# fraunhoferhhi/vvenc

Measured on AMD Instinct MI355X. Metric: frames/sec + bit-exact vs CPU, 1080p/4K 10-bit preset=faster at 1/2/4/8 GPU, higher is better.
Workload: dtype i16; 1 GPU; BASELINE configs[1]: hot-path work lists RECORDED from the reference encoder (1920x1080 10-bit synthetic clip, 65 frames, preset faster; one picture per temporal layer), replayed resident in HBM: a step = one picture's integer-ME SAD windows + sub-pel SATD stages + table calls + fused TU transform/quant lists + DMVR lists on 5 HIP streams; steps follow the GOP's 1:1:2:4:8:16 layer mix from the key; hip_streams=5, sample_pairs_per_frame=175309451, coefficients_per_frame=6951461, recorded_calls_outside_the_lists=0

## Files before the change

### vvenc_amd/csrc/me.hip

```cpp
#include <stdlib.h>
#ifndef VVHIP_ME_HU
#define VVHIP_ME_HU 2
#endif
#ifndef VVHIP_ME_STAGE_WAVES
#define VVHIP_ME_STAGE_WAVES 6
#endif
#ifndef VVHIP_ME_ITEM_WAVES
#define VVHIP_ME_ITEM_WAVES 8
#endif
#include <string.h>
#include <algorithm>
#include <vector>
#include "common.h"

struct vvhip_me_plan
{
  int bitDepth = 0, nCands = 0, nStages = 0, nItems = 0, nMaskItems = 0, maxPlane = 0;
  int wavesInt = 0, wavesStage = 0, wavesItem = 0, wavesItemMain = 0, ldsInt = 0, ldsStage = 0;
  int intBig = 0, ldsIntSmall = 0;
  int intLarge = 0, ldsIntMid = 0;
  bool stageAtomic = false;
  bool intSplit = false;
  bool timing = false; hipEvent_t ev[5] = { nullptr, nullptr, nullptr, nullptr, nullptr };
  int stageSetWaves[6] = { 0, 0, 0, 0, 0, 0 }, stageSetLds[6] = { 0, 0, 0, 0, 0, 0 };
  void* d_blob = nullptr;
  const void* d_intJobs = nullptr; const void* d_cands = nullptr; const void* d_candOut = nullptr; const void* d_stageJobs = nullptr; const void* d_stageOrder = nullptr; const void* d_stageWaves = nullptr;
  const void* d_items = nullptr; const void* d_itemOrder = nullptr; const void* d_itemWaves = nullptr; const void* d_tapTables = nullptr; const void* d_maskItems = nullptr;
};

namespace {

typedef uint32_t u32x2 __attribute__( ( ext_vector_type( 2 ) ) );
typedef uint32_t u32x4 __attribute__( ( ext_vector_type( 4 ) ) );
typedef short s16x2 __attribute__( ( ext_vector_type( 2 ) ) );
struct __attribute__( ( packed, aligned( 2 ) ) ) U8  { u32x2 v; };
struct __attribute__( ( packed, aligned( 2 ) ) ) U16 { u32x4 v; };
#define ME_GLOBAL __attribute__( ( address_space( 1 ) ) )
__device__ __forceinline__ u32x2 ld8( const int16_t* p )  { return ( ( const ME_GLOBAL U8* ) p )->v; }
__device__ __forceinline__ u32x4 ld16( const int16_t* p ) { return ( ( const ME_GLOBAL U16* ) p )->v; }
__device__ __forceinline__ u32x4 ld16o( const char* base, uint32_t byteOff ) { return reinterpret_cast<const U16*>( base + byteOff )->v; }
__device__ __forceinline__ u32x2 ld8o( const char* base, uint32_t byteOff ) { return reinterpret_cast<const U8*>( base + byteOff )->v; }
__device__ __forceinline__ int lo16( uint32_t v ) { return ( int ) ( int16_t ) ( v & 0xffffu ); }
__device__ __forceinline__ int hi16( uint32_t v ) { return ( int ) ( ( int32_t ) v >> 16 ); }
__device__ __forceinline__ uint32_t pkAdd( uint32_t a, uint32_t b ) { return __builtin_bit_cast( uint32_t, __builtin_bit_cast( s16x2, a ) + __builtin_bit_cast( s16x2, b ) ); }
__device__ __forceinline__ uint32_t pkSub( uint32_t a, uint32_t b ) { return __builtin_bit_cast( uint32_t, __builtin_bit_cast( s16x2, a ) - __builtin_bit_cast( s16x2, b ) ); }
__device__ __forceinline__ uint32_t pack2( int lo, int hi ) { return ( ( uint32_t ) lo & 0xffffu ) | ( ( uint32_t ) hi << 16 ); }
constexpr uint32_t BIAS = 0x80008000u;

struct MePlanes { const int16_t* p[16]; int stride[16]; };

struct IntJob   { int32_t orgOff, refOff; int16_t w, h; uint8_t orgPlane, refPlane, subShift, pad; int16_t minDx, minDy, winW, winH; int32_t firstCand, nCand; };
struct PlanCand { int16_t dx, dy; uint32_t out; };
struct WaveSpan { int32_t first, count; };
struct StageUnit
{
  vvhip_me_stage_job j;
  int16_t hx[3]; uint8_t nHor, nPos;
  uint8_t cnt0, cnt1, cnt2, pad;
  int32_t order;
  int32_t pos[9];
  int32_t pad2[3];
};
static_assert( sizeof( StageUnit ) == 88, "StageUnit layout" );
struct MeArgs
{
  const IntJob* intJobs; const PlanCand* cands; const int32_t* candOut; int wavesInt;
  const StageUnit* stageUnits; const WaveSpan* stageWaves; int wavesStage;
  const int32_t* tapTables;
  const vvhip_me_item* items; const int32_t* itemOrder; const WaveSpan* itemWaves; int wavesItem;
  const vvhip_me_mask_item* maskItems;
  uint64_t* candCost; uint64_t* stageCost; uint64_t* itemCost;
  int bitDepth;
};

__device__ __forceinline__ uint32_t hadamard4x4( int ( &d )[16] )
{
#pragma unroll
  for( int r = 0; r < 4; r++ )
  {
    const int a = d[4 * r], b = d[4 * r + 1], c = d[4 * r + 2], e = d[4 * r + 3];
    const int s0 = a + b, s1 = a - b, s2 = c + e, s3 = c - e;
    d[4 * r] = s0 + s2; d[4 * r + 1] = s1 + s3; d[4 * r + 2] = s0 - s2; d[4 * r + 3] = s1 - s3;
  }
  uint32_t s = 0;
#pragma unroll
  for( int c = 0; c < 4; c++ )
  {
    const int a = d[c], b = d[4 + c], e = d[8 + c], f = d[12 + c];
    const int s0 = a + b, s1 = a - b, s2 = e + f, s3 = e - f;
    const int v0 = s0 + s2, v1 = s1 + s3, v2 = s0 - s2, v3 = s1 - s3;
    s += ( c == 0 ? ( ( uint32_t ) abs( v0 ) >> 2 ) : ( uint32_t ) abs( v0 ) ) + ( uint32_t ) abs( v1 ) + ( uint32_t ) abs( v2 ) + ( uint32_t ) abs( v3 );
  }
  return ( s + 1 ) >> 1;
}

__device__ __forceinline__ int winPitch( int winW ) { return 2 * ( ( ( winW + 3 ) >> 1 ) | 1 ); }

template<bool ONE_WAVE>
__device__ __forceinline__ void intBody( const MePlanes& P, const MeArgs& a, int wave, int16_t* lds )
{
  const IntJob j = a.intJobs[wave];
  const int tid = ONE_WAVE ? ( int ) ( threadIdx.x & 63 ) : ( int ) threadIdx.x, nthr = ONE_WAVE ? 64 : ( int ) blockDim.x, lane = tid & 63;
  const int w = j.w, ss = j.subShift, rowsEff = j.h >> ss, lpr = w >> 3, lprShift = 31 - __builtin_clz( lpr );
  const int pitch = winPitch( j.winW ), half0 = ( j.winH + 1 ) >> 1;
  int16_t* win = lds;
  int16_t* orgL = lds + ( ( j.winH * pitch + 7 ) & ~7 );
  PlanCand* candL = reinterpret_cast<PlanCand*>( orgL + rowsEff * w );
  {
    PlanCand myCand = { 0, 0, 0u };
    if( tid < j.nCand ) myCand = a.cands[j.firstCand + tid];
    const char* orgB = reinterpret_cast<const char*>( P.p[j.orgPlane] + j.orgOff );
    const int os = P.stride[j.orgPlane] ? P.stride[j.orgPlane] : w, m = rowsEff * lpr;
    u32x4 ov[4]; int oat[4];
#pragma unroll
    for( int q = 0; q < 4; q++ )
    {
      const int i = tid + nthr * q < m ? tid + nthr * q : 0, r = i >> lprShift, c = i & ( lpr - 1 );
      oat[q] = r * w + c * 8;
      ov[q] = ld16o( orgB, ( uint32_t ) ( __mul24( r << ss, os ) + c * 8 ) * 2u );
    }
    const char* refB = reinterpret_cast<const char*>( P.p[j.refPlane] + j.refOff + ( ptrdiff_t ) j.minDy * P.stride[j.refPlane] + j.minDx );
    const int cpr = ( j.winW + 2 + 7 ) >> 3, n = j.winH * cpr, rs = P.stride[j.refPlane];
    const uint32_t cprInv = ( ( 1u << 20 ) + ( uint32_t ) cpr - 1u ) / ( uint32_t ) cpr;
    for( int i0 = tid; i0 < n; i0 += 4 * nthr )
    {
      u32x4 v[4]; int at[4], cc[4];
#pragma unroll
      for( int q = 0; q < 4; q++ )
      {
        const int i = i0 + nthr * q < n ? i0 + nthr * q : i0, r = ( int ) ( __umul24( ( uint32_t ) i, cprInv ) >> 20 ), c = i - __mul24( r, cpr );
        const int dr = ss ? ( ( r & 1 ) ? half0 : 0 ) + ( r >> 1 ) : r;
        at[q] = __mul24( dr, pitch ) + c * 8; cc[q] = c;
        v[q] = ld16o( refB, ( uint32_t ) ( __mul24( r, rs ) + c * 8 ) * 2u );
      }
#pragma unroll
      for( int q = 0; q < 4; q++ )
        if( i0 + nthr * q < n )
        {
          uint32_t* d = reinterpret_cast<uint32_t*>( win + at[q] );
          const int left = ( pitch >> 1 ) - cc[q] * 4;
          d[0] = v[q].x ^ BIAS; if( left > 1 ) d[1] = v[q].y ^ BIAS; if( left > 2 ) d[2] = v[q].z ^ BIAS; if( left > 3 ) d[3] = v[q].w ^ BIAS;
        }
    }
#pragma unroll
    for( int q = 0; q < 4; q++ )
      if( tid + nthr * q < m ) { u32x4 x = ov[q]; x.x ^= BIAS; x.y ^= BIAS; x.z ^= BIAS; x.w ^= BIAS; *reinterpret_cast<u32x4*>( orgL + oat[q] ) = x; }
    for( int i0 = tid + 4 * nthr; i0 < m; i0 += nthr )
    {
      const int r = i0 >> lprShift, c = i0 & ( lpr - 1 );
      u32x4 x = ld16o( orgB, ( uint32_t ) ( __mul24( r << ss, os ) + c * 8 ) * 2u ); x.x ^= BIAS; x.y ^= BIAS; x.z ^= BIAS; x.w ^= BIAS;
      *reinterpret_cast<u32x4*>( orgL + r * w + c * 8 ) = x;
    }
    if( tid < j.nCand ) candL[tid] = myCand;
    for( int i = tid + nthr; i < j.nCand; i += nthr ) candL[i] = a.cands[j.firstCand + i];
  }
  if( ONE_WAVE ) { __builtin_amdgcn_fence( __ATOMIC_ACQ_REL, "wavefront" ); __builtin_amdgcn_wave_barrier(); }
  else __syncthreads();
  const int chunks = rowsEff * lpr;
  int lpc = 64; while( lpc > chunks ) lpc >>= 1;
  const int teams = nthr / lpc, lt = tid & ( lpc - 1 ), team = tid / lpc;
  for( int c0 = 0; c0 < j.nCand; c0 += teams )
  {
    const int ci = c0 + team;
    const bool valid = ci < j.nCand;
    const PlanCand cd = candL[valid ? ci : 0];
    const int myOut = ( valid && ( uint32_t ) lt <= ( cd.out >> 24 ) ) ? a.candOut[( cd.out & 0xffffffu ) + lt] : -1;
    const int x = cd.dx - j.minDx, y = cd.dy - j.minDy;
    const int rowBase = ss ? ( ( y & 1 ) ? half0 : 0 ) + ( y >> 1 ) : y;
    const int16_t* base = win + rowBase * pitch + ( x & ~1 );
    const uint32_t sh = ( x & 1 ) * 16;
    uint32_t sad = 0;
    const uint32_t* pc = reinterpret_cast<const uint32_t*>( base + ( lt >> lprShift ) * pitch + ( lt & ( lpr - 1 ) ) * 8 );
    const u32x4* po = reinterpret_cast<const u32x4*>( orgL + ( lt >> lprShift ) * w + ( lt & ( lpr - 1 ) ) * 8 );
    const int rowStep = lpc >> lprShift, curStep = rowStep * ( pitch >> 1 ), orgStep = rowStep * ( w >> 3 );
#pragma unroll 2
    for( int it = chunks / lpc; it > 0; it-- )
    {
      const u32x4 o = *po;
      const uint32_t v0 = pc[0], v1 = pc[1], v2 = pc[2], v3 = pc[3], v4 = pc[4];
      sad = __builtin_amdgcn_sad_u16( __builtin_amdgcn_alignbit( v1, v0, sh ), o.x, sad );
      sad = __builtin_amdgcn_sad_u16( __builtin_amdgcn_alignbit( v2, v1, sh ), o.y, sad );
      sad = __builtin_amdgcn_sad_u16( __builtin_amdgcn_alignbit( v3, v2, sh ), o.z, sad );
      sad = __builtin_amdgcn_sad_u16( __builtin_amdgcn_alignbit( v4, v3, sh ), o.w, sad );
      pc += curStep; po += orgStep;
    }
    const uint32_t t = vvhipGroupSum32( sad, lpc, lane );
    if( myOut >= 0 ) a.candCost[myOut] = ( uint64_t ) t << ss;
  }
}

static const int8_t kLuma8[9][8] = {
  { 0, 0, 0, 64, 0, 0, 0, 0 }, { 0, 1, -3, 63, 4, -2, 1, 0 }, { -1, 2, -5, 62, 8, -3, 1, 0 }, { -1, 3, -8, 60, 13, -4, 1, 0 }, { -1, 4, -10, 58, 17, -5, 1, 0 },
  { -1, 4, -11, 52, 26, -8, 3, -1 }, { -1, 3, -9, 47, 31, -10, 4, -1 }, { -1, 4, -11, 45, 34, -10, 4, -1 }, { -1, 4, -11, 40, 40, -11, 4, -1 } };
static const int8_t kLuma6[9][8] = {
  { 0, 0, 0, 64, 0, 0, 0, 0 }, { 0, 1, -3, 63, 4, -2, 1, 0 }, { 0, 1, -5, 62, 8, -3, 1, 0 }, { 0, 2, -8, 60, 13, -4, 1, 0 }, { 0, 3, -10, 58, 17, -5, 1, 0 },
  { 0, 3, -11, 52, 26, -8, 2, 0 }, { 0, 2, -9, 47, 31, -10, 3, 0 }, { 0, 3, -11, 45, 34, -10, 3, 0 }, { 0, 3, -11, 40, 40, -11, 3, 0 } };
static const int8_t kAltHpel[8] = { 0, 3, 9, 20, 20, 9, 3, 0 };
static const int8_t kChroma4[17][4] = {
  { 0, 64, 0, 0 }, { -1, 63, 2, 0 }, { -2, 62, 4, 0 }, { -2, 60, 7, -1 }, { -2, 58, 10, -2 }, { -3, 57, 12, -2 }, { -4, 56, 14, -2 }, { -4, 55, 15, -2 }, { -4, 54, 16, -2 },
  { -5, 53, 18, -2 }, { -6, 52, 20, -2 }, { -6, 49, 24, -3 }, { -6, 46, 28, -4 }, { -5, 44, 29, -4 }, { -4, 42, 30, -4 }, { -4, 39, 33, -4 }, { -4, 36, 36, -4 } };

static int stageTap( int frac, int k, int filterMode, int altHpel )
{
  if( altHpel && frac == 8 ) return kAltHpel[k];
  if( filterMode == 2 )
  {
    const int ph = frac << 1;
    return ( k < 2 || k > 5 ) ? 0 : ( ph <= 16 ? kChroma4[ph][k - 2] : kChroma4[32 - ph][5 - k] );
  }
  const int p = frac <= 8 ? frac : 16 - frac, kk = frac <= 8 ? k : 7 - k;
  return filterMode == 0 ? kLuma8[p][kk] : kLuma6[p][kk];
}

static std::vector<int32_t> stageTapTables( int bitDepth )
{
  const int headRoom = 14 - bitDepth > 2 ? 14 - bitDepth : 2, vScale = 1 << ( 10 - headRoom ), hScale = 1 << ( 2 + headRoom );
  std::vector<int32_t> tapTab( 6 * 192, 0 );
  for( int mode = 0; mode < 3; mode++ ) for( int alt = 0; alt < 2; alt++ )
  {
    int32_t* t = &tapTab[( mode * 2 + alt ) * 192];
    const int set = ( mode == 2 && !alt ) ? 0 : ( mode == 0 ? 2 : 1 ), k0 = set == 0 ? 2 : ( set == 1 ? 1 : 0 ), np = set == 0 ? 2 : ( set == 1 ? 3 : 4 );
// ... 661 lines not shown
  extern __shared__ __attribute__( ( aligned( 16 ) ) ) int16_t meLds[];
  const int blk = ( int ) blockIdx.x + blockBase;
  if( blk < nBig ) { intBody<false>( P, a, blk, meLds ); return; }
  const int wv = __builtin_amdgcn_readfirstlane( ( int ) ( threadIdx.x >> 6 ) );
  const int job = nBig + ( blk - nBig ) * 4 + wv;
  if( job < a.wavesInt ) intBody<true>( P, a, job, meLds + wv * ( ldsSmall >> 1 ) );
}

template<int WAVES, bool GEN>
__global__ void __launch_bounds__( 64 * WAVES ) __attribute__( ( amdgpu_waves_per_eu( GEN ? VVHIP_ME_ITEM_WAVES - 1 : VVHIP_ME_ITEM_WAVES, GEN ? VVHIP_ME_ITEM_WAVES - 1 : VVHIP_ME_ITEM_WAVES ) ) )
meItemKernel( MePlanes P, MeArgs a, int nItems, int firstWave, int nWaves, int spansPerWave )
{
  const int wave = ( ( int ) blockIdx.x * WAVES + __builtin_amdgcn_readfirstlane( ( int ) ( threadIdx.x >> 6 ) ) ) * spansPerWave;
  for( int q = 0; q < spansPerWave; q++ )
    if( wave + q < nWaves ) { itemBody<GEN>( P, a, firstWave + wave + q, nItems ); __builtin_amdgcn_fence( __ATOMIC_ACQ_REL, "wavefront" ); __builtin_amdgcn_wave_barrier(); }
}

std::vector<int> xcdBandOrder( int nGroups, int base )
{
  std::vector<int> perm( nGroups );
  const int q = ( nGroups + 7 ) / 8;
  int cursor[8], endOf[8];
  for( int x = 0; x < 8; x++ ) { cursor[x] = std::min( nGroups, x * q ); endOf[x] = std::min( nGroups, ( x + 1 ) * q ); }
  for( int l = 0; l < nGroups; l++ )
  {
    int x = ( base + l ) & 7;
    for( int t = 0; t < 8 && cursor[x] >= endOf[x]; t++ ) x = ( x + 1 ) & 7;
    perm[l] = cursor[x]++;
  }
  return perm;
}
bool xcdBandOn() { static const bool on = !( getenv( "VVHIP_ME_XCD_BAND" ) && atoi( getenv( "VVHIP_ME_XCD_BAND" ) ) == 0 ); return on; }

int hostWinPitch( int winW ) { return 2 * ( ( ( winW + 3 ) >> 1 ) | 1 ); }
int hostWinSamples( int winW, int winH ) { return ( winH * hostWinPitch( winW ) + 7 ) & ~7; }

}

#ifndef VVHIP_ME_KERNELS_ONLY
extern "C" {

static int mePlanCreate( vvhip_ctx* ctx, const vvhip_me_lists& L, int bit_depth, int max_window, vvhip_me_plan** out );

int vvhip_get_me_tap_tables_host( int bit_depth, int32_t* host_out )
{
  if( bit_depth < 8 || bit_depth > 10 || !host_out ) return VVHIP_E_ARG;
  const std::vector<int32_t> t = stageTapTables( bit_depth );
  memcpy( host_out, t.data(), t.size() * sizeof( int32_t ) );
  return VVHIP_OK;
}

int vvhip_me_plan_create( vvhip_ctx* ctx, const vvhip_me_int_job* int_jobs, int n_int_jobs, const vvhip_me_cand* cands, int n_cands,
                          const vvhip_me_stage_job* stage_jobs, int n_stage_jobs, const vvhip_me_item* items, int n_items, int bit_depth, int max_window, vvhip_me_plan** out )
{
  vvhip_me_lists L; L.int_jobs = int_jobs; L.n_int_jobs = n_int_jobs; L.cands = cands; L.n_cands = n_cands; L.stage_jobs = stage_jobs; L.n_stage_jobs = n_stage_jobs;
  L.items = items; L.n_items = n_items; L.mask_items = nullptr; L.n_mask_items = 0;
  return mePlanCreate( ctx, L, bit_depth, max_window, out );
}

int vvhip_me_plan_create_lists( vvhip_ctx* ctx, const vvhip_me_lists* lists, int bit_depth, int max_window, vvhip_me_plan** out )
{
  if( !ctx || !lists ) return VVHIP_E_ARG;
  return mePlanCreate( ctx, *lists, bit_depth, max_window, out );
}

static int mePlanCreate( vvhip_ctx* ctx, const vvhip_me_lists& L, int bit_depth, int max_window, vvhip_me_plan** out )
{
  if( !ctx || !out ) return VVHIP_E_ARG;
  *out = nullptr;
  const vvhip_me_int_job* int_jobs = L.int_jobs; const vvhip_me_cand* cands = L.cands; const vvhip_me_stage_job* stage_jobs = L.stage_jobs; const vvhip_me_item* items = L.items;
  const vvhip_me_mask_item* mask_items = L.mask_items;
  const int n_int_jobs = L.n_int_jobs, n_cands = L.n_cands, n_stage_jobs = L.n_stage_jobs, n_items = L.n_items, n_mask = L.n_mask_items;
  if( n_int_jobs < 0 || n_cands < 0 || n_stage_jobs < 0 || n_items < 0 || n_mask < 0 || ( n_int_jobs && ( !int_jobs || !cands ) ) || ( n_stage_jobs && !stage_jobs ) || ( n_items && !items ) || ( n_mask && !mask_items ) )
    return vvhip_fail( ctx, VVHIP_E_ARG, "vvhip_me_plan_create: bad lists" );
  if( n_cands >= ( 1 << 24 ) ) return vvhip_fail( ctx, VVHIP_E_ARG, "vvhip_me_plan_create: %d candidates (the schedule packs the output-list position into 24 bits)", n_cands );
  if( n_stage_jobs > ST_STAGE_MASK ) return vvhip_fail( ctx, VVHIP_E_ARG, "vvhip_me_plan_create: %d stage jobs (the schedule packs the stage index into 22 bits)", n_stage_jobs );
  if( bit_depth < 8 || bit_depth > 10 ) return vvhip_fail( ctx, VVHIP_E_UNSUPPORTED, "vvhip_me_plan_create: bit depth %d (the packed Hadamard tile covers <= 10)", bit_depth );
  if( max_window <= 0 ) max_window = 24;
  auto shapeOk = []( int w, int h, int minW, int minH ) { return isPow2( w ) && isPow2( h ) && w >= minW && h >= minH && w <= 128 && h <= 128; };

  std::vector<IntJob> ij; std::vector<PlanCand> pc; std::vector<int32_t> candOut;
  int ldsInt = 0;
  static const bool dedupe = !( getenv( "VVHIP_ME_DEDUPE" ) && atoi( getenv( "VVHIP_ME_DEDUPE" ) ) == 0 );
  static const int candCap = getenv( "VVHIP_ME_CAND_CAP" ) ? atoi( getenv( "VVHIP_ME_CAND_CAP" ) ) : 16;
  for( int i = 0; i < n_int_jobs; i++ )
  {
    const vvhip_me_int_job& s = int_jobs[i];
    if( !shapeOk( s.width, s.height, 8, 4 ) || s.org_plane > 15 || s.ref_plane > 15 || s.sub_shift > 1 || ( s.height >> s.sub_shift ) < 1 || s.first_cand < 0 || s.n_cand < 0 || s.first_cand + s.n_cand > n_cands )
      return vvhip_fail( ctx, VVHIP_E_ARG, "vvhip_me_plan_create: integer job %d (%dx%d, candidates %d+%d)", i, s.width, s.height, s.first_cand, s.n_cand );
    struct WinCand { int16_t dx, dy; std::vector<int32_t> outs; };
    struct Win { int x0, y0, x1, y1; std::vector<WinCand> c; };
    const int teamLanes = std::min( 64, ( s.height >> s.sub_shift ) * ( s.width >> 3 ) );
    std::vector<Win> wins;
    const int reach = std::min( max_window, s.width * s.height >= 128 * 64 ? 16 : max_window );
    for( int k = 0; k < s.n_cand; k++ )
    {
      const vvhip_me_cand& c = cands[s.first_cand + k];
      WinCand p; p.dx = c.dx; p.dy = c.dy; p.outs.assign( 1, s.first_cand + k );
      bool placed = false;
      if( dedupe )
        for( Win& wn : wins )
        {
          for( WinCand& q : wn.c ) if( q.dx == c.dx && q.dy == c.dy && ( int ) q.outs.size() < teamLanes ) { q.outs.push_back( s.first_cand + k ); placed = true; break; }
          if( placed ) break;
        }
      if( placed ) continue;
      for( Win& wn : wins )
      {
        if( ( int ) wn.c.size() >= candCap ) continue;
        const int x0 = std::min( wn.x0, ( int ) c.dx ), y0 = std::min( wn.y0, ( int ) c.dy ), x1 = std::max( wn.x1, ( int ) c.dx ), y1 = std::max( wn.y1, ( int ) c.dy );
        if( x1 - x0 <= reach && y1 - y0 <= reach ) { wn.x0 = x0; wn.y0 = y0; wn.x1 = x1; wn.y1 = y1; wn.c.push_back( p ); placed = true; break; }
      }
      if( !placed ) { Win wn; wn.x0 = wn.x1 = c.dx; wn.y0 = wn.y1 = c.dy; wn.c.push_back( p ); wins.push_back( wn ); }
    }
    for( const Win& wn : wins )
    {
      IntJob j; j.orgOff = s.org_off; j.refOff = s.ref_off; j.w = s.width; j.h = s.height; j.orgPlane = s.org_plane; j.refPlane = s.ref_plane; j.subShift = s.sub_shift; j.pad = 0;
      j.minDx = ( int16_t ) wn.x0; j.minDy = ( int16_t ) wn.y0; j.winW = ( int16_t ) ( wn.x1 - wn.x0 + s.width ); j.winH = ( int16_t ) ( wn.y1 - wn.y0 + s.height );
      j.firstCand = ( int32_t ) pc.size(); j.nCand = ( int32_t ) wn.c.size();
      for( const WinCand& q : wn.c )
      {
        PlanCand pcd; pcd.dx = q.dx; pcd.dy = q.dy; pcd.out = ( uint32_t ) candOut.size() | ( uint32_t ) ( q.outs.size() - 1 ) << 24;
        pc.push_back( pcd ); candOut.insert( candOut.end(), q.outs.begin(), q.outs.end() );
      }
      ij.push_back( j );
      ldsInt = std::max( ldsInt, ( hostWinSamples( j.winW, j.winH ) + ( s.height >> s.sub_shift ) * s.width ) * 2 + j.nCand * ( int ) sizeof( PlanCand ) );
    }
  }
  auto ldsOf = []( const IntJob& j ) { return ( hostWinSamples( j.winW, j.winH ) + ( j.h >> j.subShift ) * j.w ) * 2 + j.nCand * ( int ) sizeof( PlanCand ); };
  const int ldsSmallCap = 6 * 1024, ldsMidCap = 24 * 1024;
  const bool band = xcdBandOn();
  auto classOf = [&]( const IntJob& j ) { const int l = ldsOf( j ); return l > ldsMidCap ? 0 : ( l > ldsSmallCap ? 1 : 2 ); };
  std::stable_sort( ij.begin(), ij.end(), [&]( const IntJob& a, const IntJob& b ) { const int ca = classOf( a ), cb = classOf( b ); if( ca != cb ) return ca < cb;
                    if( band ) return a.refOff < b.refOff;
                    return ( long ) a.nCand * a.w * ( a.h >> a.subShift ) + ( long ) a.winW * a.winH > ( long ) b.nCand * b.w * ( b.h >> b.subShift ) + ( long ) b.winW * b.winH; } );
  int intLarge = 0, intBig = 0, ldsIntSmall = 0, ldsIntMid = 0;
  for( const IntJob& j : ij ) { const int c = classOf( j ); if( c == 0 ) intLarge++; if( c <= 1 ) intBig++; if( c == 1 ) ldsIntMid = std::max( ldsIntMid, ldsOf( j ) ); if( c == 2 ) ldsIntSmall = std::max( ldsIntSmall, ldsOf( j ) ); }
  if( band && !ij.empty() )
  {
    auto weightOf = []( const IntJob& j ) { return ( long ) j.nCand * j.w * ( j.h >> j.subShift ) + ( long ) j.winW * j.winH; };
    auto heavyFirstPerEighth = [&]( int begin, int n, int per ) { const int q = ( ( n + per - 1 ) / per + 7 ) / 8 * per;
      for( int x = 0; x < 8 && q; x++ ) { const int a = std::min( n, x * q ), b = std::min( n, ( x + 1 ) * q );
        std::stable_sort( ij.begin() + begin + a, ij.begin() + begin + b, [&]( const IntJob& u, const IntJob& v ) { return weightOf( u ) > weightOf( v ); } ); } };
    heavyFirstPerEighth( 0, intLarge, 1 );
    heavyFirstPerEighth( intLarge, intBig - intLarge, 1 );
    heavyFirstPerEighth( intBig, ( int ) ij.size() - intBig, 4 );
    std::vector<IntJob> src( ij );
    const std::vector<int> pl = xcdBandOrder( intLarge, 0 );
    for( int l = 0; l < intLarge; l++ ) ij[l] = src[pl[l]];
    const std::vector<int> pb = xcdBandOrder( intBig - intLarge, intLarge );
    for( int l = 0; l < intBig - intLarge; l++ ) ij[intLarge + l] = src[intLarge + pb[l]];
    const int nSmall = ( int ) src.size() - intBig, nGr = ( nSmall + 3 ) / 4;
    const std::vector<int> ps = xcdBandOrder( nGr, intBig );
    for( int l = 0, o = intBig; l < nGr; l++ ) for( int k = 0; k < 4 && ps[l] * 4 + k < nSmall; k++ ) ij[o++] = src[intBig + ps[l] * 4 + k];
  }

  std::vector<WaveSpan> stWaves;
  int ldsStage = 0;
  for( int i = 0; i < n_stage_jobs; i++ )
  {
    const vvhip_me_stage_job& s = stage_jobs[i];
    bool ok = shapeOk( s.width, s.height, 4, 4 ) && !( s.width == 4 && s.height == 4 ) && s.org_plane <= 15 && s.ref_plane <= 15 && ( s.i_frac == 1 || s.i_frac == 2 ) && s.filter_mode <= 2 &&
              ( s.func == VVHIP_DF_SAD || s.func == VVHIP_DF_HAD || s.func == VVHIP_DF_HAD_FAST ) && !( s.mask >> 9 );
    for( int k = 0; ok && k < 9; k++ )
      if( ( s.mask >> k ) & 1 )
      {
        static const int8_t rxT[9] = { 0, 0, 0, -1, 1, -1, 1, -1, 1 }, ryH[9] = { 0, -1, 1, 0, 0, -1, -1, 1, 1 }, ryQ[9] = { 0, -1, 1, -1, -1, 0, 0, 1, 1 };
        const int tx = ( rxT[k] + s.base_qx ) * s.i_frac * 4, ty = ( ( s.i_frac == 2 ? ryH[k] : ryQ[k] ) + s.base_qy ) * s.i_frac * 4;
        if( tx < -16 || tx > 16 || ty < -16 || ty > 16 ) ok = false;
      }
// ... 196 lines not shown
  }

  int maxPlane = 0;
  for( int i = 0; i < n_int_jobs; i++ ) maxPlane = std::max( maxPlane, ( int ) std::max( int_jobs[i].org_plane, int_jobs[i].ref_plane ) );
  for( int i = 0; i < n_stage_jobs; i++ ) maxPlane = std::max( maxPlane, ( int ) std::max( stage_jobs[i].org_plane, stage_jobs[i].ref_plane ) );
  for( int i = 0; i < n_items; i++ ) maxPlane = std::max( maxPlane, ( int ) std::max( items[i].org_plane, items[i].cur_plane ) );
  for( int i = 0; i < n_mask; i++ ) maxPlane = std::max( maxPlane, ( int ) std::max( mask_items[i].mask_plane, std::max( mask_items[i].org_plane, mask_items[i].cur_plane ) ) );
  std::vector<StageUnit> stUnits( stOrder.size() );
  for( size_t i = 0; i < stOrder.size(); i++ )
  {
    StageUnit& u = stUnits[i];
    memset( &u, 0, sizeof( u ) );
    u.j = stage_jobs[stOrder[i] & ST_STAGE_MASK]; u.order = stOrder[i];
    static const int8_t rxT[9] = { 0, 0, 0, -1, 1, -1, 1, -1, 1 }, ryH[9] = { 0, -1, 1, 0, 0, -1, -1, 1, 1 }, ryQ[9] = { 0, -1, 1, -1, -1, 0, 0, 1, 1 };
    int tx[9], ty[9], var[9], cnt[3] = { 0, 0, 0 }, nHor = 0, nPos = 0;
    for( int k = 0; k < 9; k++ )
    {
      if( !( ( u.j.mask >> k ) & 1 ) ) continue;
      tx[k] = ( rxT[k] + u.j.base_qx ) * u.j.i_frac * 4; ty[k] = ( ( u.j.i_frac == 2 ? ryH[k] : ryQ[k] ) + u.j.base_qy ) * u.j.i_frac * 4;
      int v = 0; while( v < nHor && u.hx[v] != tx[k] ) v++;
      if( v == nHor ) u.hx[nHor++] = ( int16_t ) tx[k];
      var[k] = v; cnt[v]++; nPos++;
    }
    u.nHor = ( uint8_t ) nHor; u.nPos = ( uint8_t ) nPos; u.cnt0 = ( uint8_t ) cnt[0]; u.cnt1 = ( uint8_t ) cnt[1]; u.cnt2 = ( uint8_t ) cnt[2];
    int slot[3] = { 0, cnt[0], cnt[0] + cnt[1] };
    for( int k = 0; k < 9; k++ ) if( ( u.j.mask >> k ) & 1 ) u.pos[slot[var[k]]++] = k | ( ( tx[k] + 64 ) << 8 ) | ( ( ty[k] + 64 ) << 20 );
  }
  std::vector<vvhip_me_item> itSorted( n_items );
  for( int i = 0; i < n_items; i++ ) itSorted[i] = items[itOrder[i]];
  std::vector<vvhip_me_mask_item> mkSorted( n_mask );
  for( int i = 0; i < n_mask; i++ ) { mkSorted[i] = mask_items[itOrder[n_items + i]]; itOrder[n_items + i] += n_items; }
  const std::vector<int32_t> tapTab = stageTapTables( bit_depth );
  auto pad = []( size_t b ) { return ( b + 255 ) & ~( size_t ) 255; };
  const size_t bInt = pad( ij.size() * sizeof( IntJob ) ), bCand = pad( pc.size() * sizeof( PlanCand ) ), bCandO = pad( candOut.size() * 4 ), bSt = pad( stUnits.size() * sizeof( StageUnit ) ),
               bStO = pad( stOrder.size() * 4 ), bStW = pad( stWaves.size() * sizeof( WaveSpan ) ), bIt = pad( ( size_t ) n_items * sizeof( vvhip_me_item ) ), bItO = pad( itOrder.size() * 4 ),
               bItW = pad( itWaves.size() * sizeof( WaveSpan ) ), bMk = pad( mkSorted.size() * sizeof( vvhip_me_mask_item ) );
  const size_t bTap = pad( tapTab.size() * 4 );
  const size_t total = bInt + bCand + bCandO + bSt + bStO + bStW + bIt + bItO + bItW + bTap + bMk + 256;
  std::vector<char> host( total, 0 );
  size_t o = 0;
  auto put = [&]( const void* src, size_t bytes, size_t padded ) { const size_t at = o; if( bytes ) memcpy( host.data() + o, src, bytes ); o += padded; return at; };
  const size_t oInt = put( ij.data(), ij.size() * sizeof( IntJob ), bInt ), oCand = put( pc.data(), pc.size() * sizeof( PlanCand ), bCand ), oCandO = put( candOut.data(), candOut.size() * 4, bCandO ),
               oSt = put( stUnits.data(), stUnits.size() * sizeof( StageUnit ), bSt ), oStO = put( stOrder.data(), stOrder.size() * 4, bStO ),
               oStW = put( stWaves.data(), stWaves.size() * sizeof( WaveSpan ), bStW ), oIt = put( itSorted.data(), ( size_t ) n_items * sizeof( vvhip_me_item ), bIt ),
               oItO = put( itOrder.data(), itOrder.size() * 4, bItO ), oItW = put( itWaves.data(), itWaves.size() * sizeof( WaveSpan ), bItW ), oTap = put( tapTab.data(), tapTab.size() * 4, bTap ),
               oMk = put( mkSorted.data(), mkSorted.size() * sizeof( vvhip_me_mask_item ), bMk );
  vvhip_me_plan* p = new vvhip_me_plan;
  hipError_t e = hipMalloc( &p->d_blob, total );
  if( e != hipSuccess ) { delete p; return vvhip_fail( ctx, VVHIP_E_NOMEM, "vvhip_me_plan_create: hipMalloc( %zu ): %s", total, hipGetErrorString( e ) ); }
  e = hipMemcpyAsync( p->d_blob, host.data(), total, hipMemcpyHostToDevice, ctx->stream );
  if( e == hipSuccess ) e = hipStreamSynchronize( ctx->stream );
  if( e != hipSuccess ) { ( void ) hipFree( p->d_blob ); delete p; return vvhip_fail( ctx, VVHIP_E_HIP, "vvhip_me_plan_create: upload: %s", hipGetErrorString( e ) ); }
  char* b = static_cast<char*>( p->d_blob );
  p->d_intJobs = b + oInt; p->d_cands = b + oCand; p->d_candOut = b + oCandO; p->d_stageJobs = b + oSt; p->d_stageOrder = b + oStO; p->d_stageWaves = b + oStW; p->d_items = b + oIt; p->d_itemOrder = b + oItO; p->d_itemWaves = b + oItW; p->d_tapTables = b + oTap; p->d_maskItems = b + oMk;
  p->bitDepth = bit_depth; p->nCands = n_cands; p->nStages = n_stage_jobs; p->nItems = n_items; p->nMaskItems = n_mask; p->maxPlane = maxPlane; p->stageAtomic = hasAtomic;
  p->wavesInt = ( int ) ij.size(); p->wavesStage = ( int ) stWaves.size(); p->wavesItem = ( int ) itWaves.size(); p->wavesItemMain = wavesItemMain;
  p->ldsInt = ( ldsInt + 15 ) & ~15; p->ldsStage = ( ldsStage + 15 ) & ~15;
  for( int k = 0; k < 6; k++ ) { p->stageSetWaves[k] = setWaves[k]; p->stageSetLds[k] = setLds[k]; }
  p->intBig = intBig; p->ldsIntSmall = ( ldsIntSmall + 15 ) & ~15; p->intLarge = intLarge; p->ldsIntMid = ( ldsIntMid + 15 ) & ~15;
  p->intSplit = intBig > 0 && intBig < ( int ) ij.size() && p->ldsInt > 2 * 4 * p->ldsIntSmall && p->ldsInt > 32 * 1024;
  if( p->ldsInt > 160 * 1024 || p->ldsStage > 64 * 1024 )
  { ( void ) hipFree( p->d_blob ); delete p; return vvhip_fail( ctx, VVHIP_E_UNSUPPORTED, "vvhip_me_plan_create: %d / %d bytes of LDS per wave (max_window too large?)", ldsInt, ldsStage ); }
  *out = p;
  return VVHIP_OK;
}

void vvhip_me_plan_destroy( vvhip_ctx* ctx, vvhip_me_plan* plan )
{
  if( !plan ) return;
  if( ctx ) ( void ) hipStreamSynchronize( ctx->stream );
  if( plan->d_blob ) ( void ) hipFree( plan->d_blob );
  for( hipEvent_t e : plan->ev ) if( e ) ( void ) hipEventDestroy( e );
  delete plan;
}

int vvhip_me_plan_info( const vvhip_me_plan* plan, int* waves_int, int* waves_stage, int* waves_item, int* lds_bytes )
{
  if( !plan ) return VVHIP_E_ARG;
  if( waves_int ) *waves_int = plan->wavesInt;
  if( waves_stage ) *waves_stage = plan->wavesStage;
  if( waves_item ) *waves_item = plan->wavesItem;
  if( lds_bytes ) *lds_bytes = plan->ldsInt > plan->ldsStage ? plan->ldsInt : plan->ldsStage;
  return VVHIP_OK;
}

int vvhip_me_plan_set_timing( vvhip_ctx* ctx, vvhip_me_plan* plan, int on )
{
// ... 2 lines not shown
  plan->timing = on != 0;
  return VVHIP_OK;
}

int vvhip_me_plan_last_times( vvhip_ctx* ctx, const vvhip_me_plan* plan, float* ms4 )
{
  if( !ctx || !plan || !ms4 || !plan->timing ) return VVHIP_E_ARG;
  VVHIP_CHECK_HIP( ctx, hipEventSynchronize( plan->ev[4] ) );
  for( int k = 0; k < 4; k++ ) VVHIP_CHECK_HIP( ctx, hipEventElapsedTime( &ms4[k], plan->ev[k], plan->ev[k + 1] ) );
  return VVHIP_OK;
}

static int mePlanRun( vvhip_ctx* ctx, const vvhip_me_plan* plan, const vvhip_me_plane* planes_host, int n_planes, uint64_t* d_cand_cost, uint64_t* d_stage_cost, uint64_t* d_item_cost, int parts );

int vvhip_me_plan_run( vvhip_ctx* ctx, const vvhip_me_plan* plan, const vvhip_me_plane* planes_host, int n_planes, uint64_t* d_cand_cost, uint64_t* d_stage_cost, uint64_t* d_item_cost )
{
  return mePlanRun( ctx, plan, planes_host, n_planes, d_cand_cost, d_stage_cost, d_item_cost, 7 );
}

int vvhip_me_plan_run_parts( vvhip_ctx* ctx, const vvhip_me_plan* plan, const vvhip_me_plane* planes_host, int n_planes, uint64_t* d_cand_cost, uint64_t* d_stage_cost, uint64_t* d_item_cost, int parts )
{
  return mePlanRun( ctx, plan, planes_host, n_planes, d_cand_cost, d_stage_cost, d_item_cost, parts );
}

static int mePlanRun( vvhip_ctx* ctx, const vvhip_me_plan* plan, const vvhip_me_plane* planes_host, int n_planes, uint64_t* d_cand_cost, uint64_t* d_stage_cost, uint64_t* d_item_cost, int parts )
{
  if( !ctx || !plan ) return VVHIP_E_ARG;
  if( !planes_host || n_planes < 1 || n_planes > 16 || ( plan->nCands && !d_cand_cost ) || ( plan->nStages && !d_stage_cost ) || ( ( plan->nItems || plan->nMaskItems ) && !d_item_cost ) )
    return vvhip_fail( ctx, VVHIP_E_ARG, "vvhip_me_plan_run: bad arguments" );
  if( plan->maxPlane >= n_planes ) return vvhip_fail( ctx, VVHIP_E_ARG, "vvhip_me_plan_run: the plan's lists use plane %d, the table has %d", plan->maxPlane, n_planes );
  MePlanes P;
  for( int i = 0; i < 16; i++ ) { P.p[i] = planes_host[i < n_planes ? i : 0].d_base; P.stride[i] = planes_host[i < n_planes ? i : 0].stride; }
  MeArgs a;
  a.intJobs = static_cast<const IntJob*>( plan->d_intJobs ); a.cands = static_cast<const PlanCand*>( plan->d_cands ); a.candOut = static_cast<const int32_t*>( plan->d_candOut ); a.wavesInt = plan->wavesInt;
  a.stageUnits = static_cast<const StageUnit*>( plan->d_stageJobs );
  a.stageWaves = static_cast<const WaveSpan*>( plan->d_stageWaves ); a.wavesStage = plan->wavesStage; a.tapTables = static_cast<const int32_t*>( plan->d_tapTables );
  a.items = static_cast<const vvhip_me_item*>( plan->d_items ); a.itemOrder = static_cast<const int32_t*>( plan->d_itemOrder ); a.itemWaves = static_cast<const WaveSpan*>( plan->d_itemWaves ); a.wavesItem = plan->wavesItem;
  a.maskItems = static_cast<const vvhip_me_mask_item*>( plan->d_maskItems );
  a.candCost = d_cand_cost; a.stageCost = d_stage_cost; a.itemCost = d_item_cost; a.bitDepth = plan->bitDepth;
  const bool tm = plan->timing && parts == 7;
  const bool doStage = ( parts & 1 ) != 0, doInt = ( parts & 2 ) != 0, doItem = ( parts & 4 ) != 0;
  if( tm ) VVHIP_CHECK_HIP( ctx, hipEventRecord( plan->ev[0], ctx->stream ) );
  if( plan->stageAtomic && doStage ) VVHIP_CHECK_HIP( ctx, hipMemsetAsync( d_stage_cost, 0, ( size_t ) 9 * 8 * plan->nStages, ctx->stream ) );
  int firstWave = 0;
  static const int ldsPadExp = getenv( "VVHIP_ME_LDS_PAD" ) ? atoi( getenv( "VVHIP_ME_LDS_PAD" ) ) : 0;
  constexpr int stW = 2;
#define ME_STAGE_LAUNCH( CLS, K0, K1, GEN ) \
  if( plan->stageSetWaves[CLS] && doStage ) { const size_t ldsSt = ( ( size_t ) plan->stageSetLds[CLS] + ldsPadExp + 15 ) & ~( size_t ) 15; \
    hipLaunchKernelGGL( ( meStageKernel<K0, K1, GEN> ), dim3( ( unsigned ) ( ( plan->stageSetWaves[CLS] + stW - 1 ) / stW ) ), dim3( 64 * stW ), ( size_t ) stW * ldsSt, ctx->stream, P, a, firstWave, plan->stageSetWaves[CLS], ( int ) ldsSt ); } \
  firstWave += plan->stageSetWaves[CLS];
  ME_STAGE_LAUNCH( 0, 2, 5, false ) ME_STAGE_LAUNCH( 1, 2, 5, true )
  ME_STAGE_LAUNCH( 2, 1, 6, false ) ME_STAGE_LAUNCH( 3, 1, 6, true )
  ME_STAGE_LAUNCH( 4, 0, 7, false ) ME_STAGE_LAUNCH( 5, 0, 7, true )
#undef ME_STAGE_LAUNCH
  if( tm ) VVHIP_CHECK_HIP( ctx, hipEventRecord( plan->ev[1], ctx->stream ) );
  if( plan->wavesInt && doInt )
  {
    const int nSmall = plan->wavesInt - plan->intBig, lds = std::max( plan->intBig ? plan->ldsInt : 0, nSmall ? 4 * plan->ldsIntSmall : 0 );
    if( plan->ldsInt > 64 * 1024 ) VVHIP_CHECK_HIP( ctx, hipFuncSetAttribute( ( const void* ) meIntKernel, hipFuncAttributeMaxDynamicSharedMemorySize, plan->ldsInt ) );
    const int nLarge = plan->intLarge, nMid = plan->intBig - nLarge;
    const bool splitLarge = nLarge > 0 && nMid > 0 && plan->ldsInt > plan->ldsIntMid + plan->ldsIntMid / 2;
    const bool splitSmall = plan->intSplit;
    if( !splitLarge && !splitSmall ) hipLaunchKernelGGL( meIntKernel, dim3( ( unsigned ) ( plan->intBig + ( nSmall + 3 ) / 4 ) ), dim3( 256 ), ( size_t ) lds, ctx->stream, P, a, plan->intBig, plan->ldsIntSmall, 0 );
    else
    {
      if( splitLarge )
      {
// ... 39 lines not shown
```

Measured before the change: 15390 frames/s.

## Decouple integer-ME SAD team size from output fan-out; scatter costs via LDS

Integer-ME SAD results are now written to an LDS cost array and scattered afterwards through a separate sorted entry list, rather than each lane writing one output directly. This drops the old cap that tied duplicate-candidate fan-out to the team's lane count. The lanes-per-candidate shift is now chosen on the host per job, so small jobs with many candidates can use smaller teams and process more candidates per trip. The cost is an extra barrier, an extra LDS array, and a second gather pass that writes the outputs.

```diff
diff --git a/vvenc_amd/csrc/me.hip b/vvenc_amd/csrc/me.hip
--- a/vvenc_amd/csrc/me.hip
+++ b/vvenc_amd/csrc/me.hip
@@ -24,7 +24,7 @@
   bool timing = false; hipEvent_t ev[5] = { nullptr, nullptr, nullptr, nullptr, nullptr };
   int stageSetWaves[6] = { 0, 0, 0, 0, 0, 0 }, stageSetLds[6] = { 0, 0, 0, 0, 0, 0 };
   void* d_blob = nullptr;
-  const void* d_intJobs = nullptr; const void* d_cands = nullptr; const void* d_candOut = nullptr; const void* d_stageJobs = nullptr; const void* d_stageOrder = nullptr; const void* d_stageWaves = nullptr;
+  const void* d_intJobs = nullptr; const void* d_cands = nullptr; const void* d_ents = nullptr; const void* d_stageJobs = nullptr; const void* d_stageOrder = nullptr; const void* d_stageWaves = nullptr;
   const void* d_items = nullptr; const void* d_itemOrder = nullptr; const void* d_itemWaves = nullptr; const void* d_tapTables = nullptr; const void* d_maskItems = nullptr;
 };
 
@@ -49,8 +49,9 @@
 
 struct MePlanes { const int16_t* p[16]; int stride[16]; };
 
-struct IntJob   { int32_t orgOff, refOff; int16_t w, h; uint8_t orgPlane, refPlane, subShift, pad; int16_t minDx, minDy, winW, winH; int32_t firstCand, nCand; };
-struct PlanCand { int16_t dx, dy; uint32_t out; };
+struct IntJob   { int32_t orgOff, refOff; int16_t w, h; uint8_t orgPlane, refPlane, subShift, lpcShift; int16_t minDx, minDy, winW, winH; int32_t firstCand, nCand, firstEnt, nEnt; };
+struct PlanCand { int16_t dx, dy; };
+struct PlanEnt  { int32_t out, cand; };
 struct WaveSpan { int32_t first, count; };
 struct StageUnit
 {
@@ -64,7 +65,7 @@
 static_assert( sizeof( StageUnit ) == 88, "StageUnit layout" );
 struct MeArgs
 {
-  const IntJob* intJobs; const PlanCand* cands; const int32_t* candOut; int wavesInt;
+  const IntJob* intJobs; const PlanCand* cands; const PlanEnt* ents; int wavesInt;
   const StageUnit* stageUnits; const WaveSpan* stageWaves; int wavesStage;
   const int32_t* tapTables;
   const vvhip_me_item* items; const int32_t* itemOrder; const WaveSpan* itemWaves; int wavesItem;
@@ -94,7 +95,7 @@
   return ( s + 1 ) >> 1;
 }
 
-__device__ __forceinline__ int winPitch( int winW ) { return 2 * ( ( ( winW + 3 ) >> 1 ) | 1 ); }
+__host__ __device__ __forceinline__ int winPitch( int winW ) { return 2 * ( ( ( winW + 3 ) >> 1 ) | 1 ); }
 
 template<bool ONE_WAVE>
 __device__ __forceinline__ void intBody( const MePlanes& P, const MeArgs& a, int wave, int16_t* lds )
@@ -106,9 +107,12 @@
   int16_t* win = lds;
   int16_t* orgL = lds + ( ( j.winH * pitch + 7 ) & ~7 );
   PlanCand* candL = reinterpret_cast<PlanCand*>( orgL + rowsEff * w );
-  {
-    PlanCand myCand = { 0, 0, 0u };
+  uint32_t* costL = reinterpret_cast<uint32_t*>( candL + j.nCand );
+  PlanEnt myEnt = { -1, 0 };
+  {
+    PlanCand myCand = { 0, 0 };
     if( tid < j.nCand ) myCand = a.cands[j.firstCand + tid];
+    if( tid < j.nEnt ) myEnt = a.ents[j.firstEnt + tid];
     const char* orgB = reinterpret_cast<const char*>( P.p[j.orgPlane] + j.orgOff );
     const int os = P.stride[j.orgPlane] ? P.stride[j.orgPlane] : w, m = rowsEff * lpr;
     u32x4 ov[4]; int oat[4];
@@ -156,15 +160,13 @@
   }
   if( ONE_WAVE ) { __builtin_amdgcn_fence( __ATOMIC_ACQ_REL, "wavefront" ); __builtin_amdgcn_wave_barrier(); }
   else __syncthreads();
-  const int chunks = rowsEff * lpr;
-  int lpc = 64; while( lpc > chunks ) lpc >>= 1;
-  const int teams = nthr / lpc, lt = tid & ( lpc - 1 ), team = tid / lpc;
+  const int chunks = rowsEff * lpr, lpcShift = j.lpcShift, lpc = 1 << lpcShift;
+  const int teams = nthr >> lpcShift, lt = tid & ( lpc - 1 ), team = tid >> lpcShift;
   for( int c0 = 0; c0 < j.nCand; c0 += teams )
   {
     const int ci = c0 + team;
     const bool valid = ci < j.nCand;
     const PlanCand cd = candL[valid ? ci : 0];
-    const int myOut = ( valid && ( uint32_t ) lt <= ( cd.out >> 24 ) ) ? a.candOut[( cd.out & 0xffffffu ) + lt] : -1;
     const int x = cd.dx - j.minDx, y = cd.dy - j.minDy;
     const int rowBase = ss ? ( ( y & 1 ) ? half0 : 0 ) + ( y >> 1 ) : y;
     const int16_t* base = win + rowBase * pitch + ( x & ~1 );
@@ -174,7 +176,7 @@
     const u32x4* po = reinterpret_cast<const u32x4*>( orgL + ( lt >> lprShift ) * w + ( lt & ( lpr - 1 ) ) * 8 );
     const int rowStep = lpc >> lprShift, curStep = rowStep * ( pitch >> 1 ), orgStep = rowStep * ( w >> 3 );
 #pragma unroll 2
-    for( int it = chunks / lpc; it > 0; it-- )
+    for( int it = chunks >> lpcShift; it > 0; it-- )
     {
       const u32x4 o = *po;
       const uint32_t v0 = pc[0], v1 = pc[1], v2 = pc[2], v3 = pc[3], v4 = pc[4];
@@ -185,8 +187,12 @@
       pc += curStep; po += orgStep;
     }
     const uint32_t t = vvhipGroupSum32( sad, lpc, lane );
-    if( myOut >= 0 ) a.candCost[myOut] = ( uint64_t ) t << ss;
-  }
+    if( valid && lt == 0 ) costL[ci] = t;
+  }
+  if( ONE_WAVE ) { __builtin_amdgcn_fence( __ATOMIC_ACQ_REL, "wavefront" ); __builtin_amdgcn_wave_barrier(); }
+  else __syncthreads();
+  if( myEnt.out >= 0 ) a.candCost[myEnt.out] = ( uint64_t ) costL[myEnt.cand] << ss;
+  for( int e = tid + nthr; e < j.nEnt; e += nthr ) { const PlanEnt en = a.ents[j.firstEnt + e]; a.candCost[en.out] = ( uint64_t ) costL[en.cand] << ss; }
 }
 
 static const int8_t kLuma8[9][8] = {
@@ -914,8 +920,7 @@
 }
 bool xcdBandOn() { static const bool on = !( getenv( "VVHIP_ME_XCD_BAND" ) && atoi( getenv( "VVHIP_ME_XCD_BAND" ) ) == 0 ); return on; }
 
-int hostWinPitch( int winW ) { return 2 * ( ( ( winW + 3 ) >> 1 ) | 1 ); }
-int hostWinSamples( int winW, int winH ) { return ( winH * hostWinPitch( winW ) + 7 ) & ~7; }
+int hostWinSamples( int winW, int winH ) { return ( winH * winPitch( winW ) + 7 ) & ~7; }
 
 }
 
@@ -961,7 +966,7 @@
   if( max_window <= 0 ) max_window = 24;
   auto shapeOk = []( int w, int h, int minW, int minH ) { return isPow2( w ) && isPow2( h ) && w >= minW && h >= minH && w <= 128 && h <= 128; };
 
-  std::vector<IntJob> ij; std::vector<PlanCand> pc; std::vector<int32_t> candOut;
+  std::vector<IntJob> ij; std::vector<PlanCand> pc; std::vector<PlanEnt> ents;
   int ldsInt = 0;
   static const bool dedupe = !( getenv( "VVHIP_ME_DEDUPE" ) && atoi( getenv( "VVHIP_ME_DEDUPE" ) ) == 0 );
   static const int candCap = getenv( "VVHIP_ME_CAND_CAP" ) ? atoi( getenv( "VVHIP_ME_CAND_CAP" ) ) : 16;
@@ -972,7 +977,6 @@
       return vvhip_fail( ctx, VVHIP_E_ARG, "vvhip_me_plan_create: integer job %d (%dx%d, candidates %d+%d)", i, s.width, s.height, s.first_cand, s.n_cand );
     struct WinCand { int16_t dx, dy; std::vector<int32_t> outs; };
     struct Win { int x0, y0, x1, y1; std::vector<WinCand> c; };
-    const int teamLanes = std::min( 64, ( s.height >> s.sub_shift ) * ( s.width >> 3 ) );
     std::vector<Win> wins;
     const int reach = std::min( max_window, s.width * s.height >= 128 * 64 ? 16 : max_window );
     for( int k = 0; k < s.n_cand; k++ )
@@ -983,7 +987,7 @@
       if( dedupe )
         for( Win& wn : wins )
         {
-          for( WinCand& q : wn.c ) if( q.dx == c.dx && q.dy == c.dy && ( int ) q.outs.size() < teamLanes ) { q.outs.push_back( s.first_cand + k ); placed = true; break; }
+          for( WinCand& q : wn.c ) if( q.dx == c.dx && q.dy == c.dy ) { q.outs.push_back( s.first_cand + k ); placed = true; break; }
           if( placed ) break;
         }
       if( placed ) continue;
@@ -997,27 +1001,48 @@
     }
     for( const Win& wn : wins )
     {
-      IntJob j; j.orgOff = s.org_off; j.refOff = s.ref_off; j.w = s.width; j.h = s.height; j.orgPlane = s.org_plane; j.refPlane = s.ref_plane; j.subShift = s.sub_shift; j.pad = 0;
+      IntJob j; j.orgOff = s.org_off; j.refOff = s.ref_off; j.w = s.width; j.h = s.height; j.orgPlane = s.org_plane; j.refPlane = s.ref_plane; j.subShift = s.sub_shift;
       j.minDx = ( int16_t ) wn.x0; j.minDy = ( int16_t ) wn.y0; j.winW = ( int16_t ) ( wn.x1 - wn.x0 + s.width ); j.winH = ( int16_t ) ( wn.y1 - wn.y0 + s.height );
-      j.firstCand = ( int32_t ) pc.size(); j.nCand = ( int32_t ) wn.c.size();
-      for( const WinCand& q : wn.c )
-      {
-        PlanCand pcd; pcd.dx = q.dx; pcd.dy = q.dy; pcd.out = ( uint32_t ) candOut.size() | ( uint32_t ) ( q.outs.size() - 1 ) << 24;
-        pc.push_back( pcd ); candOut.insert( candOut.end(), q.outs.begin(), q.outs.end() );
-      }
+      j.firstCand = ( int32_t ) pc.size(); j.nCand = ( int32_t ) wn.c.size(); j.firstEnt = ( int32_t ) ents.size(); j.lpcShift = 0;
+      for( int q = 0; q < j.nCand; q++ )
+      {
+        PlanCand pcd; pcd.dx = wn.c[q].dx; pcd.dy = wn.c[q].dy; pc.push_back( pcd );
+        for( int32_t o : wn.c[q].outs ) { PlanEnt en; en.out = o; en.cand = q; ents.push_back( en ); }
+      }
+      std::sort( ents.begin() + j.firstEnt, ents.end(), []( const PlanEnt& a, const PlanEnt& b ) { return a.out < b.out; } );
+      j.nEnt = ( int32_t ) ents.size() - j.firstEnt;
       ij.push_back( j );
-      ldsInt = std::max( ldsInt, ( hostWinSamples( j.winW, j.winH ) + ( s.height >> s.sub_shift ) * s.width ) * 2 + j.nCand * ( int ) sizeof( PlanCand ) );
-    }
-  }
-  auto ldsOf = []( const IntJob& j ) { return ( hostWinSamples( j.winW, j.winH ) + ( j.h >> j.subShift ) * j.w ) * 2 + j.nCand * ( int ) sizeof( PlanCand ); };
+      ldsInt = std::max( ldsInt, ( hostWinSamples( j.winW, j.winH ) + ( s.height >> s.sub_shift ) * s.width ) * 2 + j.nCand * ( int ) ( sizeof( PlanCand ) + sizeof( uint32_t ) ) );
+    }
+  }
+  auto ldsOf = []( const IntJob& j ) { return ( hostWinSamples( j.winW, j.winH ) + ( j.h >> j.subShift ) * j.w ) * 2 + j.nCand * ( int ) ( sizeof( PlanCand ) + sizeof( uint32_t ) ); };
   const int ldsSmallCap = 6 * 1024, ldsMidCap = 24 * 1024;
   const bool band = xcdBandOn();
   auto classOf = [&]( const IntJob& j ) { const int l = ldsOf( j ); return l > ldsMidCap ? 0 : ( l > ldsSmallCap ? 1 : 2 ); };
   std::stable_sort( ij.begin(), ij.end(), [&]( const IntJob& a, const IntJob& b ) { const int ca = classOf( a ), cb = classOf( b ); if( ca != cb ) return ca < cb;
                     if( band ) return a.refOff < b.refOff;
                     return ( long ) a.nCand * a.w * ( a.h >> a.subShift ) + ( long ) a.winW * a.winH > ( long ) b.nCand * b.w * ( b.h >> b.subShift ) + ( long ) b.winW * b.winH; } );
+  int teamTrips = 1, teamFloor = 1;
+#ifdef VVHIP_DEV_KNOBS
+  if( getenv( "VVHIP_ME_INT_TRIPS" ) ) teamTrips = std::max( 1, atoi( getenv( "VVHIP_ME_INT_TRIPS" ) ) );
+  if( getenv( "VVHIP_ME_INT_LPC_MIN" ) ) teamFloor = std::max( 1, atoi( getenv( "VVHIP_ME_INT_LPC_MIN" ) ) );
+#endif
+  auto teamShiftOf = [&]( const IntJob& j, int nthr ) { const int lpr = j.w >> 3, chunks = ( j.h >> j.subShift ) * lpr;
+    int cp2 = 1; while( cp2 * teamTrips < j.nCand ) cp2 <<= 1;
+    int lpc = std::max( std::max( 1, nthr / cp2 ), teamFloor ); while( !isPow2( lpc ) ) lpc &= lpc - 1;
+    return ilog2i( std::max( lpr, std::min( lpc, std::min( 64, chunks ) ) ) ); };
+  for( IntJob& j : ij ) j.lpcShift = ( uint8_t ) teamShiftOf( j, classOf( j ) == 2 ? 64 : 256 );
   int intLarge = 0, intBig = 0, ldsIntSmall = 0, ldsIntMid = 0;
   for( const IntJob& j : ij ) { const int c = classOf( j ); if( c == 0 ) intLarge++; if( c <= 1 ) intBig++; if( c == 1 ) ldsIntMid = std::max( ldsIntMid, ldsOf( j ) ); if( c == 2 ) ldsIntSmall = std::max( ldsIntSmall, ldsOf( j ) ); }
+#ifdef VVHIP_DEV_KNOBS
+  if( getenv( "VVHIP_ME_INT_REPORT" ) )
+  {
+    long trips = 0, cands = 0;
+    for( const IntJob& j : ij ) { const int teams = ( classOf( j ) == 2 ? 64 : 256 ) >> j.lpcShift; trips += ( j.nCand + teams - 1 ) / teams; cands += j.nCand; }
+    fprintf( stderr, "vvhip_me_plan_create: windows %d = %d (> 24 KB) + %d (> 6 KB) + %d (one wave), LDS %d / %d / %d, %ld candidates, %d entries, %ld trips\n", ( int ) ij.size(), intLarge, intBig - intLarge,
+             ( int ) ij.size() - intBig, ldsInt, ldsIntMid, ldsIntSmall, cands, ( int ) ents.size(), trips );
+  }
+#endif
   if( band && !ij.empty() )
   {
     auto weightOf = []( const IntJob& j ) { return ( long ) j.nCand * j.w * ( j.h >> j.subShift ) + ( long ) j.winW * j.winH; };
@@ -1280,15 +1305,15 @@
   for( int i = 0; i < n_mask; i++ ) { mkSorted[i] = mask_items[itOrder[n_items + i]]; itOrder[n_items + i] += n_items; }
   const std::vector<int32_t> tapTab = stageTapTables( bit_depth );
   auto pad = []( size_t b ) { return ( b + 255 ) & ~( size_t ) 255; };
-  const size_t bInt = pad( ij.size() * sizeof( IntJob ) ), bCand = pad( pc.size() * sizeof( PlanCand ) ), bCandO = pad( candOut.size() * 4 ), bSt = pad( stUnits.size() * sizeof( StageUnit ) ),
+  const size_t bInt = pad( ij.size() * sizeof( IntJob ) ), bCand = pad( pc.size() * sizeof( PlanCand ) ), bEnt = pad( ents.size() * sizeof( PlanEnt ) ), bSt = pad( stUnits.size() * sizeof( StageUnit ) ),
                bStO = pad( stOrder.size() * 4 ), bStW = pad( stWaves.size() * sizeof( WaveSpan ) ), bIt = pad( ( size_t ) n_items * sizeof( vvhip_me_item ) ), bItO = pad( itOrder.size() * 4 ),
                bItW = pad( itWaves.size() * sizeof( WaveSpan ) ), bMk = pad( mkSorted.size() * sizeof( vvhip_me_mask_item ) );
   const size_t bTap = pad( tapTab.size() * 4 );
-  const size_t total = bInt + bCand + bCandO + bSt + bStO + bStW + bIt + bItO + bItW + bTap + bMk + 256;
+  const size_t total = bInt + bCand + bEnt + bSt + bStO + bStW + bIt + bItO + bItW + bTap + bMk + 256;
   std::vector<char> host( total, 0 );
   size_t o = 0;
   auto put = [&]( const void* src, size_t bytes, size_t padded ) { const size_t at = o; if( bytes ) memcpy( host.data() + o, src, bytes ); o += padded; return at; };
-  const size_t oInt = put( ij.data(), ij.size() * sizeof( IntJob ), bInt ), oCand = put( pc.data(), pc.size() * sizeof( PlanCand ), bCand ), oCandO = put( candOut.data(), candOut.size() * 4, bCandO ),
+  const size_t oInt = put( ij.data(), ij.size() * sizeof( IntJob ), bInt ), oCand = put( pc.data(), pc.size() * sizeof( PlanCand ), bCand ), oEnt = put( ents.data(), ents.size() * sizeof( PlanEnt ), bEnt ),
                oSt = put( stUnits.data(), stUnits.size() * sizeof( StageUnit ), bSt ), oStO = put( stOrder.data(), stOrder.size() * 4, bStO ),
                oStW = put( stWaves.data(), stWaves.size() * sizeof( WaveSpan ), bStW ), oIt = put( itSorted.data(), ( size_t ) n_items * sizeof( vvhip_me_item ), bIt ),
                oItO = put( itOrder.data(), itOrder.size() * 4, bItO ), oItW = put( itWaves.data(), itWaves.size() * sizeof( WaveSpan ), bItW ), oTap = put( tapTab.data(), tapTab.size() * 4, bTap ),
@@ -1300,7 +1325,7 @@
   if( e == hipSuccess ) e = hipStreamSynchronize( ctx->stream );
   if( e != hipSuccess ) { ( void ) hipFree( p->d_blob ); delete p; return vvhip_fail( ctx, VVHIP_E_HIP, "vvhip_me_plan_create: upload: %s", hipGetErrorString( e ) ); }
   char* b = static_cast<char*>( p->d_blob );
-  p->d_intJobs = b + oInt; p->d_cands = b + oCand; p->d_candOut = b + oCandO; p->d_stageJobs = b + oSt; p->d_stageOrder = b + oStO; p->d_stageWaves = b + oStW; p->d_items = b + oIt; p->d_itemOrder = b + oItO; p->d_itemWaves = b + oItW; p->d_tapTables = b + oTap; p->d_maskItems = b + oMk;
+  p->d_intJobs = b + oInt; p->d_cands = b + oCand; p->d_ents = b + oEnt; p->d_stageJobs = b + oSt; p->d_stageOrder = b + oStO; p->d_stageWaves = b + oStW; p->d_items = b + oIt; p->d_itemOrder = b + oItO; p->d_itemWaves = b + oItW; p->d_tapTables = b + oTap; p->d_maskItems = b + oMk;
   p->bitDepth = bit_depth; p->nCands = n_cands; p->nStages = n_stage_jobs; p->nItems = n_items; p->nMaskItems = n_mask; p->maxPlane = maxPlane; p->stageAtomic = hasAtomic;
   p->wavesInt = ( int ) ij.size(); p->wavesStage = ( int ) stWaves.size(); p->wavesItem = ( int ) itWaves.size(); p->wavesItemMain = wavesItemMain;
   p->ldsInt = ( ldsInt + 15 ) & ~15; p->ldsStage = ( ldsStage + 15 ) & ~15;
@@ -1369,7 +1394,7 @@
   MePlanes P;
   for( int i = 0; i < 16; i++ ) { P.p[i] = planes_host[i < n_planes ? i : 0].d_base; P.stride[i] = planes_host[i < n_planes ? i : 0].stride; }
   MeArgs a;
-  a.intJobs = static_cast<const IntJob*>( plan->d_intJobs ); a.cands = static_cast<const PlanCand*>( plan->d_cands ); a.candOut = static_cast<const int32_t*>( plan->d_candOut ); a.wavesInt = plan->wavesInt;
+  a.intJobs = static_cast<const IntJob*>( plan->d_intJobs ); a.cands = static_cast<const PlanCand*>( plan->d_cands ); a.ents = static_cast<const PlanEnt*>( plan->d_ents ); a.wavesInt = plan->wavesInt;
   a.stageUnits = static_cast<const StageUnit*>( plan->d_stageJobs );
   a.stageWaves = static_cast<const WaveSpan*>( plan->d_stageWaves ); a.wavesStage = plan->wavesStage; a.tapTables = static_cast<const int32_t*>( plan->d_tapTables );
   a.items = static_cast<const vvhip_me_item*>( plan->d_items ); a.itemOrder = static_cast<const int32_t*>( plan->d_itemOrder ); a.itemWaves = static_cast<const WaveSpan*>( plan->d_itemWaves ); a.wavesItem = plan->wavesItem;
```

Result: no change. 15560 frames/s (median of 4 runs) (+1.1%).
